# anuragranj/cc

Measured on NVIDIA H100. Metric: train-step triplets/sec at 256x832x6lvl, higher is better.
Workload: dtype f32

## Files before the change

### cc_b200/csrc/conv_tc.cu

```cuda
#include "conv.cuh"

#ifndef CCB_CPU_SIM

#include <cuda.h>
#include <cudaTypedefs.h>

namespace ccb {

constexpr int TC_M = 128;
constexpr int TC_NMAX = 128;
constexpr int TC_KC = 8;
constexpr int TC_MAX_STAGES = 4;
constexpr int TC_PRODUCERS = 128;
constexpr int TC_CONSUMER_WARPS = 8;
constexpr int TC_THREADS = TC_PRODUCERS + 32 * TC_CONSUMER_WARPS;
constexpr int TC_MAX_TAPS = 49;
constexpr int TC_PRODUCER_REGS = 72, TC_CONSUMER_REGS = 216;

struct TcArgs {
    CUtensorMap wmap;
    const float* x;
    const float* bias;
    const float* res;
    float* out;
// ... 33 lines not shown
        "}"
        : "=r"(ok)
        : "r"(smem_u32(bar)), "r"(parity)
        : "memory");
    return ok != 0;
}
__device__ __forceinline__ void mbar_wait(uint64_t* bar, uint32_t parity) {
    uint32_t spins = 0;
    while (!mbar_try(bar, parity)) {
        if (++spins > (1u << 26)) asm volatile("trap;");
    }
}
__device__ __forceinline__ void fence_proxy_async() { asm volatile("fence.proxy.async.shared::cta;" ::: "memory"); }
__device__ __forceinline__ void fence_barrier_init() { asm volatile("fence.mbarrier_init.release.cluster;" ::: "memory"); }
__device__ __forceinline__ void mbar_arrive_expect_tx(uint64_t* bar, uint32_t bytes) {
    asm volatile("mbarrier.arrive.expect_tx.shared::cta.b64 _, [%0], %1;" ::"r"(smem_u32(bar)), "r"(bytes) : "memory");
}
__device__ __forceinline__ void tma_load_3d(void* dst, const CUtensorMap* map, uint64_t* bar, int c0, int c1, int c2) {
    asm volatile(
        "cp.async.bulk.tensor.3d.shared::cluster.global.mbarrier::complete_tx::bytes [%0], [%1, {%3, %4, %5}], [%2];"
        ::"r"(smem_u32(dst)), "l"(map), "r"(smem_u32(bar)), "r"(c0), "r"(c1), "r"(c2)
        : "memory");
}
__device__ __forceinline__ void tma_prefetch_map(const CUtensorMap* map) {
    asm volatile("prefetch.tensormap [%0];" ::"l"(map) : "memory");
}
__device__ __forceinline__ void cp_async_4(uint32_t dst, const float* src, bool valid) {
    asm volatile("cp.async.ca.shared.global [%0], [%1], 4, %2;" ::"r"(dst), "l"(src), "r"(valid ? 4 : 0) : "memory");
}
__device__ __forceinline__ void cp_async_arrive(uint64_t* bar) {
    asm volatile("cp.async.mbarrier.arrive.noinc.shared::cta.b64 [%0];" ::"r"(smem_u32(bar)) : "memory");
}
__device__ __forceinline__ void cp_async_wait_all() { asm volatile("cp.async.wait_all;" ::: "memory"); }
__device__ __forceinline__ float tf32_hi(float x) {
    uint32_t r;
    asm("cvt.rna.tf32.f32 %0, %1;" : "=r"(r) : "f"(x));
    return __uint_as_float(r);
}

__device__ __forceinline__ uint64_t wg_desc(uint32_t saddr) {
    return (uint64_t)((saddr & 0x3FFFF) >> 4) | ((uint64_t)1 << 16) | ((uint64_t)(1024 >> 4) << 32) | ((uint64_t)1 << 62);
}
__device__ __forceinline__ void wg_fence() { asm volatile("wgmma.fence.sync.aligned;" ::: "memory"); }
__device__ __forceinline__ void wg_commit() { asm volatile("wgmma.commit_group.sync.aligned;" ::: "memory"); }
template <int PENDING>
__device__ __forceinline__ void wg_wait() { asm volatile("wgmma.wait_group.sync.aligned %0;" ::"n"(PENDING) : "memory"); }
template <int R>
__device__ __forceinline__ void wg_fence_regs(float (&d)[R]) {
#pragma unroll
    for (int i = 0; i < R; ++i) asm volatile("" : "+f"(d[i])::"memory");
}
template <int K, int R>
__device__ __forceinline__ void wg_fence_regs(uint32_t (&d)[K][R]) {
#pragma unroll
    for (int k = 0; k < K; ++k)
#pragma unroll
        for (int i = 0; i < R; ++i) asm volatile("" : "+r"(d[k][i])::"memory");
}

__device__ __forceinline__ void wgmma_tf32_n16(float (&d)[8], uint64_t da, uint64_t db) {
    asm volatile(
        "{\n\t.reg .pred p;\n\tsetp.ne.b32 p, 1, 0;\n\t"
        "wgmma.mma_async.sync.aligned.m64n16k8.f32.tf32.tf32 "
        "{%0, %1, %2, %3, %4, %5, %6, %7}, "
        "%8, %9, p, 1, 1;\n\t}"
        : "+f"(d[0]), "+f"(d[1]), "+f"(d[2]), "+f"(d[3]), "+f"(d[4]), "+f"(d[5]), "+f"(d[6]), "+f"(d[7])
        : "l"(da), "l"(db));
}
__device__ __forceinline__ void wgmma_tf32_n32(float (&d)[16], uint64_t da, uint64_t db) {
    asm volatile(
        "{\n\t.reg .pred p;\n\tsetp.ne.b32 p, 1, 0;\n\t"
        "wgmma.mma_async.sync.aligned.m64n32k8.f32.tf32.tf32 "
        "{%0, %1, %2, %3, %4, %5, %6, %7, %8, %9, %10, %11, %12, %13, %14, %15}, "
        "%16, %17, p, 1, 1;\n\t}"
        : "+f"(d[0]), "+f"(d[1]), "+f"(d[2]), "+f"(d[3]), "+f"(d[4]), "+f"(d[5]), "+f"(d[6]), "+f"(d[7]),
          "+f"(d[8]), "+f"(d[9]), "+f"(d[10]), "+f"(d[11]), "+f"(d[12]), "+f"(d[13]), "+f"(d[14]), "+f"(d[15])
        : "l"(da), "l"(db));
}
__device__ __forceinline__ void wgmma_tf32_n64(float (&d)[32], uint64_t da, uint64_t db) {
    asm volatile(
        "{\n\t.reg .pred p;\n\tsetp.ne.b32 p, 1, 0;\n\t"
        "wgmma.mma_async.sync.aligned.m64n64k8.f32.tf32.tf32 "
        "{%0, %1, %2, %3, %4, %5, %6, %7, %8, %9, %10, %11, %12, %13, %14, %15,"
        " %16, %17, %18, %19, %20, %21, %22, %23, %24, %25, %26, %27, %28, %29, %30, %31}, "
        "%32, %33, p, 1, 1;\n\t}"
        : "+f"(d[0]), "+f"(d[1]), "+f"(d[2]), "+f"(d[3]), "+f"(d[4]), "+f"(d[5]), "+f"(d[6]), "+f"(d[7]),
          "+f"(d[8]), "+f"(d[9]), "+f"(d[10]), "+f"(d[11]), "+f"(d[12]), "+f"(d[13]), "+f"(d[14]), "+f"(d[15]),
          "+f"(d[16]), "+f"(d[17]), "+f"(d[18]), "+f"(d[19]), "+f"(d[20]), "+f"(d[21]), "+f"(d[22]), "+f"(d[23]),
          "+f"(d[24]), "+f"(d[25]), "+f"(d[26]), "+f"(d[27]), "+f"(d[28]), "+f"(d[29]), "+f"(d[30]), "+f"(d[31])
        : "l"(da), "l"(db));
}
__device__ __forceinline__ void wgmma_tf32_n128(float (&d)[64], uint64_t da, uint64_t db) {
    asm volatile(
        "{\n\t.reg .pred p;\n\tsetp.ne.b32 p, 1, 0;\n\t"
        "wgmma.mma_async.sync.aligned.m64n128k8.f32.tf32.tf32 "
        "{%0, %1, %2, %3, %4, %5, %6, %7, %8, %9, %10, %11, %12, %13, %14, %15,"
        " %16, %17, %18, %19, %20, %21, %22, %23, %24, %25, %26, %27, %28, %29, %30, %31,"
        " %32, %33, %34, %35, %36, %37, %38, %39, %40, %41, %42, %43, %44, %45, %46, %47,"
        " %48, %49, %50, %51, %52, %53, %54, %55, %56, %57, %58, %59, %60, %61, %62, %63}, "
        "%64, %65, p, 1, 1;\n\t}"
        : "+f"(d[0]), "+f"(d[1]), "+f"(d[2]), "+f"(d[3]), "+f"(d[4]), "+f"(d[5]), "+f"(d[6]), "+f"(d[7]),
          "+f"(d[8]), "+f"(d[9]), "+f"(d[10]), "+f"(d[11]), "+f"(d[12]), "+f"(d[13]), "+f"(d[14]), "+f"(d[15]),
          "+f"(d[16]), "+f"(d[17]), "+f"(d[18]), "+f"(d[19]), "+f"(d[20]), "+f"(d[21]), "+f"(d[22]), "+f"(d[23]),
          "+f"(d[24]), "+f"(d[25]), "+f"(d[26]), "+f"(d[27]), "+f"(d[28]), "+f"(d[29]), "+f"(d[30]), "+f"(d[31]),
          "+f"(d[32]), "+f"(d[33]), "+f"(d[34]), "+f"(d[35]), "+f"(d[36]), "+f"(d[37]), "+f"(d[38]), "+f"(d[39]),
          "+f"(d[40]), "+f"(d[41]), "+f"(d[42]), "+f"(d[43]), "+f"(d[44]), "+f"(d[45]), "+f"(d[46]), "+f"(d[47]),
          "+f"(d[48]), "+f"(d[49]), "+f"(d[50]), "+f"(d[51]), "+f"(d[52]), "+f"(d[53]), "+f"(d[54]), "+f"(d[55]),
          "+f"(d[56]), "+f"(d[57]), "+f"(d[58]), "+f"(d[59]), "+f"(d[60]), "+f"(d[61]), "+f"(d[62]), "+f"(d[63])
        : "l"(da), "l"(db));
}
template <int NT>
__device__ __forceinline__ void wgmma_tf32(float (&d)[NT / 2], uint64_t da, uint64_t db) {
    if constexpr (NT == 16) wgmma_tf32_n16(d, da, db);
    else if constexpr (NT == 32) wgmma_tf32_n32(d, da, db);
    else if constexpr (NT == 64) wgmma_tf32_n64(d, da, db);
    else wgmma_tf32_n128(d, da, db);
}

__device__ __forceinline__ void wgmma_tf32_rs_n16(float (&d)[8], const uint32_t (&a)[4], uint64_t db) {
    asm volatile(
        "{\n\t.reg .pred p;\n\tsetp.ne.b32 p, 1, 0;\n\t"
        "wgmma.mma_async.sync.aligned.m64n16k8.f32.tf32.tf32 "
        "{%0, %1, %2, %3, %4, %5, %6, %7}, "
        "{%8, %9, %10, %11}, %12, p, 1, 1;\n\t}"
        : "+f"(d[0]), "+f"(d[1]), "+f"(d[2]), "+f"(d[3]), "+f"(d[4]), "+f"(d[5]), "+f"(d[6]), "+f"(d[7])
        : "r"(a[0]), "r"(a[1]), "r"(a[2]), "r"(a[3]), "l"(db));
}
__device__ __forceinline__ void wgmma_tf32_rs_n32(float (&d)[16], const uint32_t (&a)[4], uint64_t db) {
    asm volatile(
        "{\n\t.reg .pred p;\n\tsetp.ne.b32 p, 1, 0;\n\t"
        "wgmma.mma_async.sync.aligned.m64n32k8.f32.tf32.tf32 "
        "{%0, %1, %2, %3, %4, %5, %6, %7, %8, %9, %10, %11, %12, %13, %14, %15}, "
        "{%16, %17, %18, %19}, %20, p, 1, 1;\n\t}"
        : "+f"(d[0]), "+f"(d[1]), "+f"(d[2]), "+f"(d[3]), "+f"(d[4]), "+f"(d[5]), "+f"(d[6]), "+f"(d[7]),
          "+f"(d[8]), "+f"(d[9]), "+f"(d[10]), "+f"(d[11]), "+f"(d[12]), "+f"(d[13]), "+f"(d[14]), "+f"(d[15])
        : "r"(a[0]), "r"(a[1]), "r"(a[2]), "r"(a[3]), "l"(db));
}
__device__ __forceinline__ void wgmma_tf32_rs_n64(float (&d)[32], const uint32_t (&a)[4], uint64_t db) {
    asm volatile(
        "{\n\t.reg .pred p;\n\tsetp.ne.b32 p, 1, 0;\n\t"
        "wgmma.mma_async.sync.aligned.m64n64k8.f32.tf32.tf32 "
        "{%0, %1, %2, %3, %4, %5, %6, %7, %8, %9, %10, %11, %12, %13, %14, %15,"
        " %16, %17, %18, %19, %20, %21, %22, %23, %24, %25, %26, %27, %28, %29, %30, %31}, "
        "{%32, %33, %34, %35}, %36, p, 1, 1;\n\t}"
        : "+f"(d[0]), "+f"(d[1]), "+f"(d[2]), "+f"(d[3]), "+f"(d[4]), "+f"(d[5]), "+f"(d[6]), "+f"(d[7]),
          "+f"(d[8]), "+f"(d[9]), "+f"(d[10]), "+f"(d[11]), "+f"(d[12]), "+f"(d[13]), "+f"(d[14]), "+f"(d[15]),
          "+f"(d[16]), "+f"(d[17]), "+f"(d[18]), "+f"(d[19]), "+f"(d[20]), "+f"(d[21]), "+f"(d[22]), "+f"(d[23]),
          "+f"(d[24]), "+f"(d[25]), "+f"(d[26]), "+f"(d[27]), "+f"(d[28]), "+f"(d[29]), "+f"(d[30]), "+f"(d[31])
        : "r"(a[0]), "r"(a[1]), "r"(a[2]), "r"(a[3]), "l"(db));
// ... 50 lines not shown

    template <typename T>
    __device__ __forceinline__ TcTiles<T> tiles(T base, int s) const {
        const T st = base + s * stage_bytes;
        return {st, st + TC_TILE_BYTES, st + 2 * TC_TILE_BYTES, st + 2 * TC_TILE_BYTES + b_tile_bytes};
    }
    __device__ __forceinline__ TcTiles<unsigned char*> acquire(int it, int s) const {
        if (it >= depth) mbar_wait(&empty[s], ((it / depth) - 1) & 1);
        return tiles(smem, s);
    }
    __device__ __forceinline__ void publish(int s) const { fence_proxy_async(); mbar_arrive(&full[s]); }
};

__device__ __forceinline__ TcRing tc_ring(int depth, int b_tile_bytes, int full_arrivals) {
    CCB_PDL_TRIGGER();
    extern __shared__ __align__(1024) unsigned char smem_raw[];
    unsigned char* smem = smem_raw + ((1024u - (smem_u32(smem_raw) & 1023u)) & 1023u);
    const int stage_bytes = 2 * TC_TILE_BYTES + 2 * b_tile_bytes;
    uint64_t* full = (uint64_t*)(smem + depth * stage_bytes);
    const TcRing r = {smem, depth, stage_bytes, b_tile_bytes, full, full + TC_MAX_STAGES};
    if (threadIdx.x == 0) {
        for (int s = 0; s < depth; ++s) { mbar_init(&r.full[s], full_arrivals); mbar_init(&r.empty[s], TC_CONSUMER_WARPS); }
        fence_barrier_init();
    }
    __syncthreads();
    CCB_PDL_SYNC();
    return r;
}

__device__ __forceinline__ int tc_acc_row(int wg, int wq, int lane, int half) { return wg * 64 + wq * 16 + (lane >> 2) + half * 8; }
__device__ __forceinline__ int tc_acc_col(int lane, int i, int e) { return 8 * i + 2 * (lane & 3) + e; }
__device__ __forceinline__ int tc_acc_reg(int i, int half, int e) { return 4 * i + 2 * half + e; }

template <int NT>
__device__ __forceinline__ void tc_consume(const TcRing& ring, int nkt, int wg, int lane, float (&acc)[NT / 2]) {
    float part[NT / 2];
#pragma unroll
    for (int j = 0; j < NT / 2; ++j) acc[j] = 0.f;
    const uint32_t base = smem_u32(ring.smem);
    for (int it = 0; it < nkt; ++it) {
        const int s = it % ring.depth;
        mbar_wait(&ring.full[s], (it / ring.depth) & 1);
        const TcTiles<uint32_t> t = ring.tiles(base, s);
        const uint32_t a_hi = t.a_hi + wg * (TC_TILE_BYTES / 2), a_lo = t.a_lo + wg * (TC_TILE_BYTES / 2);
#pragma unroll
        for (int j = 0; j < NT / 2; ++j) part[j] = 0.f;
        wg_fence();
#pragma unroll
        for (int ks = 0; ks < TC_KC / 2; ++ks) {
            const uint32_t koff = (uint32_t)ks * 32u;
            wgmma_tf32<NT>(part, wg_desc(a_lo + koff), wg_desc(t.b_hi + koff));
            wgmma_tf32<NT>(part, wg_desc(a_hi + koff), wg_desc(t.b_lo + koff));
        }
#pragma unroll
        for (int ks = 0; ks < TC_KC / 2; ++ks) {
            const uint32_t koff = (uint32_t)ks * 32u;
            wgmma_tf32<NT>(part, wg_desc(a_hi + koff), wg_desc(t.b_hi + koff));
        }
        wg_commit();
        wg_wait<0>();
        wg_fence_regs(part);
        if (lane == 0) mbar_arrive(&ring.empty[s]);
#pragma unroll
        for (int j = 0; j < NT / 2; ++j) acc[j] += part[j];
    }
}

struct TcAFrag { uint32_t hi[TC_KC / 2][4], lo[TC_KC / 2][4]; };

__device__ __forceinline__ int tc_a_idx(int r, int k) { return k * TC_M + (r ^ (8 * (k & 3))); }
__device__ __forceinline__ int tc_a_off(int r0, int t) { return tc_a_idx(r0, t) * 4; }
__device__ __forceinline__ void tc_load_a(const unsigned char* tile, int off, float (&v)[2][8]) {
#pragma unroll
    for (int h = 0; h < 2; ++h)
#pragma unroll
        for (int j = 0; j < 8; ++j) v[h][j] = *(const float*)(tile + ((off ^ (32 * h)) + 2048 * j));
}
__device__ __forceinline__ void tc_split_a(const float (&v)[2][8], TcAFrag& f) {
#pragma unroll
    for (int ks = 0; ks < TC_KC / 2; ++ks)
#pragma unroll
        for (int i = 0; i < 4; ++i) {
            const float x = v[i & 1][2 * ks + (i >> 1)], h = tf32_hi(x);
            f.hi[ks][i] = __float_as_uint(h);
            f.lo[ks][i] = __float_as_uint(tf32_hi(x - h));
        }
}

template <int NT>
__device__ __forceinline__ void tc_consume_rs(const TcRing& ring, int g, int nkt, int wg, int wq, int lane, float (&acc)[NT / 2]) {
    constexpr bool split_ahead = NT < 128;
    float part[NT / 2];
#pragma unroll
    for (int j = 0; j < NT / 2; ++j) acc[j] = 0.f;
    const uint32_t base = smem_u32(ring.smem);
    const int a_off = tc_a_off(wg * 64 + wq * 16 + (lane >> 2), lane & 3);
    TcAFrag cur, nxt;
    float v[2][8];
    int s = g % ring.depth;
    uint32_t phase = (g / ring.depth) & 1;
    if constexpr (split_ahead) {
        if (nkt > 0) {
            mbar_wait(&ring.full[s], phase);
            tc_load_a(ring.tiles(ring.smem, s).a_hi, a_off, v);
            tc_split_a(v, cur);
        }
    }
    for (int it = 0; it < nkt; ++it) {
        if constexpr (!split_ahead) {
            mbar_wait(&ring.full[s], phase);
            tc_load_a(ring.tiles(ring.smem, s).a_hi, a_off, v);
            tc_split_a(v, cur);
        }
        const TcTiles<uint32_t> tl = ring.tiles(base, s);
#pragma unroll
        for (int j = 0; j < NT / 2; ++j) part[j] = 0.f;
        wg_fence();
#pragma unroll
        for (int ks = 0; ks < TC_KC / 2; ++ks) {
            const uint32_t koff = (uint32_t)ks * 32u;
            wgmma_tf32_rs<NT>(part, cur.lo[ks], wg_desc(tl.b_hi + koff));
            wgmma_tf32_rs<NT>(part, cur.hi[ks], wg_desc(tl.b_lo + koff));
        }
#pragma unroll
        for (int ks = 0; ks < TC_KC / 2; ++ks)
            wgmma_tf32_rs<NT>(part, cur.hi[ks], wg_desc(tl.b_hi + (uint32_t)ks * 32u));
        wg_commit();
        const int s1 = s + 1 == ring.depth ? 0 : s + 1;
        const uint32_t phase1 = phase ^ (s1 == 0);
        if constexpr (split_ahead) {
            if (it + 1 < nkt) {
                mbar_wait(&ring.full[s1], phase1);
                tc_load_a(ring.tiles(ring.smem, s1).a_hi, a_off, v);
                tc_split_a(v, nxt);
            }
        }
        wg_wait<0>();
        wg_fence_regs(part);
        wg_fence_regs(cur.hi);
        wg_fence_regs(cur.lo);
        if (lane == 0) mbar_arrive(&ring.empty[s]);
#pragma unroll
        for (int j = 0; j < NT / 2; ++j) acc[j] += part[j];
        if constexpr (split_ahead) cur = nxt;
        s = s1;
        phase = phase1;
    }
}

struct TcUnit { int m0, n0, z, kt_beg, nkt; };
__device__ __forceinline__ TcUnit tc_unit(const TcArgs& a, int u) {
    TcUnit w;
    w.m0 = (u % a.tiles_m) * TC_M;
    u /= a.tiles_m;
    w.n0 = (u % a.tiles_n) * TC_NMAX;
    w.z = u / a.tiles_n;
    w.kt_beg = w.z * a.kt_per_split;
    w.nkt = max(0, min(a.ktiles, w.kt_beg + a.kt_per_split) - w.kt_beg);
    return w;
}

template <int NT>
__global__ void __launch_bounds__(TC_THREADS, 1) conv_tc_kernel(const __grid_constant__ TcArgs a) {
    const TcRing ring = tc_ring(a.depth, a.b_tile_bytes, TC_PRODUCERS + 1);
    const int tid = threadIdx.x, warp = tid >> 5, lane = tid & 31;
    const long long HWin = (long long)a.Hin * a.Win;

    if (warp < TC_PRODUCERS / 32) {
        wg_regs_dec<TC_PRODUCER_REGS>();
        const int r = tid;
        const int cpt = a.cpad >> 2;
        const int nchunks = a.ntaps * cpt;
        if (r == 0) tma_prefetch_map(&a.wmap);
        int g = 0;
        for (int u = blockIdx.x; u < a.units; u += gridDim.x) {
            const TcUnit w = tc_unit(a, u);
            const int m = w.m0 + r;
            const bool mvalid = m < a.M;
            int b = 0, oy = 0, ox = 0;
            if (mvalid) {
                int hw = a.Hc * a.Wc;
                b = m / hw;
                int rem = m - b * hw;
                oy = rem / a.Wc;
// ... 35 lines not shown
#pragma unroll
                    for (int c = 0; c < TC_KC; ++c) {
                        const float* p = a.x;
                        int nv = 0;
                        if (mvalid && q < nchunks) {
                            const int iy = iy0 + a.off_y[tap], ix = ix0 + a.off_x[tap];
                            if (iy >= 0 && iy < a.Hin && ix >= 0 && ix < a.Win) {
                                p = xb + (long long)(c4 * 4) * HWin + (iy * a.Win + ix);
                                nv = a.Cin - c4 * 4;
                            }
                        }
#pragma unroll
                        for (int j = 0; j < 4; ++j) {
                            const bool v = j < nv;
                            cp_async_4(at + 4 * tc_a_idx(r, 4 * c + j), v ? p + j * HWin : a.x, v);
                        }
                        ++q;
                        if (++c4 == cpt) { c4 = 0; ++tap; }
                    }
                }
                cp_async_arrive(&ring.full[s]);
            }
        }
        cp_async_wait_all();
    } else {
        wg_regs_inc<TC_CONSUMER_REGS>();
        const int wg = (warp - TC_PRODUCERS / 32) >> 2, wq = warp & 3;
        const long long HWout = (long long)a.Hout * a.Wout;
        int g = 0;
        for (int u = blockIdx.x; u < a.units; u += gridDim.x) {
            const TcUnit w = tc_unit(a, u);
            const int ntile = min(TC_NMAX, a.Ntot - w.n0);
            float acc[NT / 2];
            tc_consume_rs<NT>(ring, g, w.nkt, wg, wq, lane, acc);
            g += w.nkt;
#pragma unroll
            for (int half = 0; half < 2; ++half) {
                const int em = w.m0 + tc_acc_row(wg, wq, lane, half);
                if (em >= a.M) continue;
                int hw = a.Hc * a.Wc;
                int eb = em / hw;
                int rem = em - eb * hw;
                int eoy = rem / a.Wc, eox = rem - eoy * a.Wc;
                const long long obase = (long long)eb * a.Ntot * HWout + (long long)(eoy * a.out_stride + a.out_oy) * a.Wout +
                                        (eox * a.out_stride + a.out_ox);
#pragma unroll
                for (int i = 0; i < NT / 8; ++i)
#pragma unroll
                    for (int e = 0; e < 2; ++e) {
                        const int nl = tc_acc_col(lane, i, e);
                        if (nl < ntile) {
                            float o = acc[tc_acc_reg(i, half, e)];
                            const int n = w.n0 + nl;
                            const long long off = obase + (long long)n * HWout;
                            if (a.splits > 1) {
                                a.partial[(long long)w.z * a.out_numel + off] = o;
                            } else {
                                if (a.bias) o += __ldg(a.bias + n);
                                if (a.res) o += __ldg(a.res + off);
                                a.out[off] = apply_act(o, a.act, a.slope);
                            }
                        }
                    }
            }
        }
    }
}
// ... 13 lines not shown
}

template <typename Args>
static int tc_launch_kernel(void (*const (&kfns)[4])(const Args), const Args& a, int nt, dim3 grid, int smem, cudaStream_t st,
                            const char* what) {
    auto kfn = kfns[nt == 16 ? 0 : nt == 32 ? 1 : nt == 64 ? 2 : 3];
    cudaFuncSetAttribute(kfn, cudaFuncAttributeMaxDynamicSharedMemorySize, TC_SMEM_MAX);
    CCB_LAUNCH(kfn, grid, dim3(TC_THREADS), smem, st, a);
    return check_launch(what);
}

static void (*const TC_FPROP_KERNELS[4])(const TcArgs) = {conv_tc_kernel<16>, conv_tc_kernel<32>, conv_tc_kernel<64>,
                                                          conv_tc_kernel<128>};

static int tc_weight_map(CUtensorMap* map, const float* wp, int N, int Kp, int nt) {
    static PFN_cuTensorMapEncodeTiled_v12000 encode = [] {
        void* fn = nullptr;
        cudaDriverEntryPointQueryResult q;
        if (cudaGetDriverEntryPointByVersion("cuTensorMapEncodeTiled", &fn, 12000, cudaEnableDefault, &q) != cudaSuccess ||
            q != cudaDriverEntryPointSuccess)
            fn = nullptr;
        return (PFN_cuTensorMapEncodeTiled_v12000)fn;
    }();
    CCB_REQUIRE(encode, CCB_ERR_LAUNCH, "conv_tc: the driver has no cuTensorMapEncodeTiled");
    const cuuint64_t dims[3] = {(cuuint64_t)Kp, (cuuint64_t)N, 2};
    const cuuint64_t strides[2] = {(cuuint64_t)Kp * sizeof(float), (cuuint64_t)N * Kp * sizeof(float)};
    const cuuint32_t box[3] = {TC_KC * 4, (cuuint32_t)nt, 1};
    const cuuint32_t estrides[3] = {1, 1, 1};
    const CUresult rc = encode(map, CU_TENSOR_MAP_DATA_TYPE_FLOAT32, 3, (void*)wp, dims, strides, box, estrides,
                               CU_TENSOR_MAP_INTERLEAVE_NONE, CU_TENSOR_MAP_SWIZZLE_128B, CU_TENSOR_MAP_L2_PROMOTION_L2_256B,
                               CU_TENSOR_MAP_FLOAT_OOB_FILL_NONE);
    CCB_REQUIRE(rc == CUDA_SUCCESS, CCB_ERR_LAUNCH, "conv_tc: cuTensorMapEncodeTiled failed (%d) for N %d Kp %d", (int)rc, N, Kp);
    return CCB_OK;
}

static int launch_tc(TcArgs& a, const float* w, int mode, int N, int Cc, int KK, int Ci, const signed char* tap_index,
                     float* wp, float* partial, int splits, cudaStream_t st) {
    a.cpad = roundup(Cc, 4);
    a.Kp = tc_kp(a.ntaps, Cc);
    WPrepDesc p;
    memset(&p, 0, sizeof(p));
    p.w = w; p.wp = wp; p.N = N; p.Cc = Cc; p.KK = KK; p.ntaps = a.ntaps; p.Kp = a.Kp; p.mode = mode; p.Ci = Ci;
    p.layout = WPREP_TC; p.p0 = a.cpad;
    for (int t = 0; t < a.ntaps; ++t) p.tap_index[t] = tap_index[t];
    const float* wpp = nullptr;
    int rc = wprep_get(p, st, &wpp);
    if (rc) return rc;
    a.Ntot = N;
    a.splits = splits;
    a.ktiles = a.Kp / (TC_KC * 4);
    a.kt_per_split = cdiv(a.ktiles, splits);
    a.partial = partial;
    int nt, smem;
    tc_geometry(N, nt, a.b_tile_bytes, a.depth, smem);
    rc = tc_weight_map(&a.wmap, wpp, N, a.Kp, nt);
    if (rc) return rc;
    a.tiles_m = cdiv(a.M, TC_M);
    a.tiles_n = cdiv(N, TC_NMAX);
    a.units = a.tiles_m * a.tiles_n * splits;
    static int sms = [] {
        int dev = 0, n = 0;
        cudaGetDevice(&dev);
        cudaDeviceGetAttribute(&n, cudaDevAttrMultiProcessorCount, dev);
        return n > 0 ? n : NUM_SMS;
    }();
    return tc_launch_kernel(TC_FPROP_KERNELS, a, nt, dim3(a.units < sms ? a.units : sms), smem, st, "conv_tc");
}

struct TcWgradArgs {
    const float* x;
    const float* dy;
    float* out;
    int B, Ci, Hi, Wi, Co, Ho, Wo, kh, kw, stride, pad;
    int cpad, Mtot;
    int P;
    int ktiles, kt_per_split, splits;
    int depth, b_tile_bytes;
};

template <int NT>
__global__ void __launch_bounds__(TC_THREADS, 1) conv_tc_wgrad_kernel(const TcWgradArgs a) {
    const TcRing ring = tc_ring(a.depth, a.b_tile_bytes, TC_PRODUCERS);
    const int tid = threadIdx.x, warp = tid >> 5, lane = tid & 31;
    const int m0 = blockIdx.x * TC_M, n0 = blockIdx.y * TC_NMAX;
    const int ntile = min(TC_NMAX, a.Co - n0);
    const int kt_beg = blockIdx.z * a.kt_per_split;
    const int nkt = min(a.ktiles, kt_beg + a.kt_per_split) - kt_beg;
    const int KK = a.kh * a.kw;
    const int HWo = a.Ho * a.Wo, HWi = a.Hi * a.Wi;

    if (warp < TC_PRODUCERS / 32) {
        const int c = tid & 7, rbase = tid >> 3;
        int rowoff[8], dky[8], dkx[8];
        unsigned rvalid = 0;
#pragma unroll
        for (int j = 0; j < 8; ++j) {
            int m = m0 + rbase + 16 * j;
            rowoff[j] = 0; dky[j] = dkx[j] = 0;
            if (m < a.Mtot) {
                int tap = m / a.cpad, ci = m - tap * a.cpad;
                if (ci < a.Ci) {
                    int ky = tap / a.kw, kx = tap - ky * a.kw;
                    dky[j] = ky - a.pad; dkx[j] = kx - a.pad;
                    rowoff[j] = ci * HWi + dky[j] * a.Wi + dkx[j];
                    rvalid |= 1u << j;
                }
            }
        }
        for (int it = 0; it < nkt; ++it) {
            const int s = it % ring.depth;
            const int p0 = ((kt_beg + it) * TC_KC + c) * 4;
            const bool pvalid = p0 < a.P;
            int b = 0, oy = 0, ox0 = 0;
            if (pvalid) {
                b = p0 / HWo;
                int rem = p0 - b * HWo;
                oy = rem / a.Wo;
                ox0 = rem - oy * a.Wo;
            }
            const float* xpix = a.x + (long long)b * a.Ci * HWi + (oy * a.stride) * a.Wi + ox0 * a.stride;
            const int iyb = oy * a.stride, ixb = ox0 * a.stride;
            float av[8][4];
            float4 bv[8];
#pragma unroll
            for (int j = 0; j < 8; ++j) {
                av[j][0] = av[j][1] = av[j][2] = av[j][3] = 0.f;
                const int iy = iyb + dky[j], ix0 = ixb + dkx[j];
                if (pvalid && ((rvalid >> j) & 1u) && iy >= 0 && iy < a.Hi) {
                    const float* px = xpix + rowoff[j];
                    if (ix0 >= 0 && ix0 + 3 * a.stride < a.Wi) {
#pragma unroll
                        for (int e = 0; e < 4; ++e) av[j][e] = __ldg(px + e * a.stride);
                    } else {
#pragma unroll
                        for (int e = 0; e < 4; ++e) {
                            const int ix = ix0 + e * a.stride;
                            if (ix >= 0 && ix < a.Wi) av[j][e] = __ldg(px + e * a.stride);
                        }
                    }
                }
                bv[j] = make_float4(0.f, 0.f, 0.f, 0.f);
                const int n = rbase + 16 * j;
                if (pvalid && n < ntile)
                    bv[j] = __ldg((const float4*)(a.dy + ((long long)b * a.Co + n0 + n) * HWo + oy * a.Wo + ox0));
            }
            const TcTiles<unsigned char*> t = ring.acquire(it, s);
#pragma unroll
            for (int j = 0; j < 8; ++j) {
                const int r = rbase + 16 * j, idx = tile_idx(r, c);
                tc_split_store(t.a_hi, t.a_lo, idx, make_float4(av[j][0], av[j][1], av[j][2], av[j][3]));
                if (r < NT) tc_split_store(t.b_hi, t.b_lo, idx, bv[j]);
            }
            ring.publish(s);
        }
    } else {
        const int wg = (warp - TC_PRODUCERS / 32) >> 2, wq = warp & 3;
        float acc[NT / 2];
        tc_consume<NT>(ring, nkt, wg, lane, acc);
        float* outp = a.out + (long long)blockIdx.z * a.Co * a.Ci * KK;
#pragma unroll
        for (int half = 0; half < 2; ++half) {
            const int em = m0 + tc_acc_row(wg, wq, lane, half);
            if (em >= a.Mtot) continue;
            const int etap = em / a.cpad;
            const int eci = em - etap * a.cpad;
            if (eci >= a.Ci) continue;
#pragma unroll
            for (int i = 0; i < NT / 8; ++i)
#pragma unroll
                for (int e = 0; e < 2; ++e) {
                    const int nl = tc_acc_col(lane, i, e);
                    if (nl < ntile) outp[((long long)(n0 + nl) * a.Ci + eci) * KK + etap] = acc[tc_acc_reg(i, half, e)];
                }
        }
    }
}

static void (*const TC_WGRAD_KERNELS[4])(const TcWgradArgs) = {conv_tc_wgrad_kernel<16>, conv_tc_wgrad_kernel<32>,
                                                                conv_tc_wgrad_kernel<64>, conv_tc_wgrad_kernel<128>};

bool tc_supported(const ccb_conv_desc* d, int op) {
    if (d->kh != d->kw || d->kh * d->kw > TC_MAX_TAPS) return false;
    if (op == CCB_CONV_WGRAD) return (d->Wo % 4 == 0);
    return true;
}
bool tc_profitable(const ccb_conv_desc* d, int op) {
    if (!tc_supported(d, op)) return false;
    const long long M = (op == CCB_CONV_FPROP) ? (long long)d->B * d->Ho * d->Wo : (long long)d->B * d->Hi * d->Wi;
    const long long wsize = (long long)d->Ci * d->Co * d->kh * d->kw;
    return (M >= 128 && wsize >= 64) || (M >= 8 && wsize >= 65536);
}

int tc_plan(const ccb_conv_desc* d, int op, long long& panel_floats) {
    panel_floats = 0;
    if (op == CCB_CONV_WGRAD) {
        const int ktiles = cdiv(d->B * d->Ho * d->Wo, 32);
        const int tiles = cdiv(d->kh * d->kw * roundup(d->Ci, 4), TC_M) * cdiv(d->Co, TC_NMAX);
        int splits = cdiv(2 * NUM_SMS, tiles);
        if (splits > ktiles / 4) splits = ktiles / 4;
        if (splits > 2 * NUM_SMS) splits = 2 * NUM_SMS;
        if (splits < 1) splits = 1;
        return cdiv(ktiles, cdiv(ktiles, splits));
    }
    const bool fp = op == CCB_CONV_FPROP;
    const int s = fp ? 1 : d->stride, N = fp ? d->Co : d->Ci;
    const int Kp = tc_kp(cdiv(d->kh, s) * cdiv(d->kw, s), fp ? d->Ci : d->Co);
// ... 56 lines not shown
            for (int ty = 0; ty < k.nky; ++ty)
                for (int tx = 0; tx < k.nkx; ++tx) {
                    const int ky = k.ky0 + ty * s, kx = k.kx0 + tx * s, t = ty * k.nkx + tx;
                    a.off_y[t] = (signed char)((py + d->pad - ky) / s);
                    a.off_x[t] = (signed char)((px + d->pad - kx) / s);
                    tix[t] = (signed char)(ky * d->kw + kx);
                }
            int rc = launch_tc(a, w, 1, d->Ci, d->Co, d->kh * d->kw, d->Ci, tix, wp, partial, splits, st);
            if (rc) return rc;
        }
    if (splits > 1) {
        launch_splitk_reduce(partial, dx, bias, res, out_numel, splits, d->Hi * d->Wi, d->Ci, d->act, d->slope, st);
        return check_launch("conv_tc dgrad splitk reduce");
    }
    return CCB_OK;
}

int tc_wgrad(const ccb_conv_desc* d, const float* x, const float* dy, float* dw, float* partial, int splits, cudaStream_t st) {
    TcWgradArgs a;
    memset(&a, 0, sizeof(a));
    a.x = x; a.dy = dy;
    a.B = d->B; a.Ci = d->Ci; a.Hi = d->Hi; a.Wi = d->Wi; a.Co = d->Co; a.Ho = d->Ho; a.Wo = d->Wo;
    a.kh = d->kh; a.kw = d->kw; a.stride = d->stride; a.pad = d->pad;
    a.cpad = roundup(d->Ci, 4);
    a.Mtot = d->kh * d->kw * a.cpad;
    a.P = d->B * d->Ho * d->Wo;
    a.ktiles = cdiv(a.P, 32);
    a.kt_per_split = cdiv(a.ktiles, splits);
    a.splits = splits;
    a.out = splits > 1 ? partial : dw;
    const long long numel = (long long)d->Co * d->Ci * d->kh * d->kw;
    int nt, wsmem;
    tc_geometry(d->Co, nt, a.b_tile_bytes, a.depth, wsmem);
    dim3 grid(cdiv(a.Mtot, TC_M), cdiv(d->Co, TC_NMAX), a.splits);
    int rc = tc_launch_kernel(TC_WGRAD_KERNELS, a, nt, grid, wsmem, st, "conv_tc_wgrad");
    if (rc || a.splits == 1) return rc;
    launch_splitk_reduce(partial, dw, nullptr, nullptr, numel, splits, 1, 1, CCB_ACT_NONE, 0.f, st);
    return check_launch("conv_tc_wgrad_reduce");
}

}

extern "C" int ccb_debug_tc_plan(int N, int* out4) {
    if (N < 1 || !out4) return CCB_ERR_ARG;
    ccb::tc_geometry(N, out4[0], out4[1], out4[2], out4[3]);
    return CCB_OK;
}

#else

namespace ccb {
bool tc_supported(const ccb_conv_desc*, int) { return false; }
bool tc_profitable(const ccb_conv_desc*, int) { return false; }
int tc_plan(const ccb_conv_desc*, int, long long& panel_floats) { panel_floats = 0; return 1; }
int tc_fprop(const ccb_conv_desc*, const float*, const float*, const float*, const float*, float*, float*, float*, int,
             cudaStream_t) { return CCB_ERR_UNSUPPORTED; }
int tc_dgrad(const ccb_conv_desc*, const float*, const float*, const float*, const float*, float*, float*, float*, int,
             cudaStream_t) { return CCB_ERR_UNSUPPORTED; }
int tc_wgrad(const ccb_conv_desc*, const float*, const float*, float*, float*, int, cudaStream_t) { return CCB_ERR_UNSUPPORTED; }
}

extern "C" int ccb_debug_tc_plan(int, int*) { return CCB_ERR_UNSUPPORTED; }

#endif
```

Measured before the change: 57.89.

## Make wgrad TC kernel persistent with cp.async producers and register-sourced A splitting

```diff
diff --git a/cc_b200/csrc/conv_tc.cu b/cc_b200/csrc/conv_tc.cu
--- a/cc_b200/csrc/conv_tc.cu
+++ b/cc_b200/csrc/conv_tc.cu
@@ -89,6 +89,9 @@
     asm volatile("cp.async.mbarrier.arrive.noinc.shared::cta.b64 [%0];" ::"r"(smem_u32(bar)) : "memory");
 }
 __device__ __forceinline__ void cp_async_wait_all() { asm volatile("cp.async.wait_all;" ::: "memory"); }
+__device__ __forceinline__ void cp_async_16(uint32_t dst, const void* src, bool valid) {
+    asm volatile("cp.async.cg.shared.global [%0], [%1], 16, %2;" ::"r"(dst), "l"(src), "r"(valid ? 16 : 0) : "memory");
+}
 __device__ __forceinline__ float tf32_hi(float x) {
     uint32_t r;
     asm("cvt.rna.tf32.f32 %0, %1;" : "=r"(r) : "f"(x));
@@ -113,65 +116,6 @@
     for (int k = 0; k < K; ++k)
 #pragma unroll
         for (int i = 0; i < R; ++i) asm volatile("" : "+r"(d[k][i])::"memory");
-}
-
-__device__ __forceinline__ void wgmma_tf32_n16(float (&d)[8], uint64_t da, uint64_t db) {
-    asm volatile(
-        "{\n\t.reg .pred p;\n\tsetp.ne.b32 p, 1, 0;\n\t"
-        "wgmma.mma_async.sync.aligned.m64n16k8.f32.tf32.tf32 "
-        "{%0, %1, %2, %3, %4, %5, %6, %7}, "
-        "%8, %9, p, 1, 1;\n\t}"
-        : "+f"(d[0]), "+f"(d[1]), "+f"(d[2]), "+f"(d[3]), "+f"(d[4]), "+f"(d[5]), "+f"(d[6]), "+f"(d[7])
-        : "l"(da), "l"(db));
-}
-__device__ __forceinline__ void wgmma_tf32_n32(float (&d)[16], uint64_t da, uint64_t db) {
-    asm volatile(
-        "{\n\t.reg .pred p;\n\tsetp.ne.b32 p, 1, 0;\n\t"
-        "wgmma.mma_async.sync.aligned.m64n32k8.f32.tf32.tf32 "
-        "{%0, %1, %2, %3, %4, %5, %6, %7, %8, %9, %10, %11, %12, %13, %14, %15}, "
-        "%16, %17, p, 1, 1;\n\t}"
-        : "+f"(d[0]), "+f"(d[1]), "+f"(d[2]), "+f"(d[3]), "+f"(d[4]), "+f"(d[5]), "+f"(d[6]), "+f"(d[7]),
-          "+f"(d[8]), "+f"(d[9]), "+f"(d[10]), "+f"(d[11]), "+f"(d[12]), "+f"(d[13]), "+f"(d[14]), "+f"(d[15])
-        : "l"(da), "l"(db));
-}
-__device__ __forceinline__ void wgmma_tf32_n64(float (&d)[32], uint64_t da, uint64_t db) {
-    asm volatile(
-        "{\n\t.reg .pred p;\n\tsetp.ne.b32 p, 1, 0;\n\t"
-        "wgmma.mma_async.sync.aligned.m64n64k8.f32.tf32.tf32 "
-        "{%0, %1, %2, %3, %4, %5, %6, %7, %8, %9, %10, %11, %12, %13, %14, %15,"
-        " %16, %17, %18, %19, %20, %21, %22, %23, %24, %25, %26, %27, %28, %29, %30, %31}, "
-        "%32, %33, p, 1, 1;\n\t}"
-        : "+f"(d[0]), "+f"(d[1]), "+f"(d[2]), "+f"(d[3]), "+f"(d[4]), "+f"(d[5]), "+f"(d[6]), "+f"(d[7]),
-          "+f"(d[8]), "+f"(d[9]), "+f"(d[10]), "+f"(d[11]), "+f"(d[12]), "+f"(d[13]), "+f"(d[14]), "+f"(d[15]),
-          "+f"(d[16]), "+f"(d[17]), "+f"(d[18]), "+f"(d[19]), "+f"(d[20]), "+f"(d[21]), "+f"(d[22]), "+f"(d[23]),
-          "+f"(d[24]), "+f"(d[25]), "+f"(d[26]), "+f"(d[27]), "+f"(d[28]), "+f"(d[29]), "+f"(d[30]), "+f"(d[31])
-        : "l"(da), "l"(db));
-}
-__device__ __forceinline__ void wgmma_tf32_n128(float (&d)[64], uint64_t da, uint64_t db) {
-    asm volatile(
-        "{\n\t.reg .pred p;\n\tsetp.ne.b32 p, 1, 0;\n\t"
-        "wgmma.mma_async.sync.aligned.m64n128k8.f32.tf32.tf32 "
-        "{%0, %1, %2, %3, %4, %5, %6, %7, %8, %9, %10, %11, %12, %13, %14, %15,"
-        " %16, %17, %18, %19, %20, %21, %22, %23, %24, %25, %26, %27, %28, %29, %30, %31,"
-        " %32, %33, %34, %35, %36, %37, %38, %39, %40, %41, %42, %43, %44, %45, %46, %47,"
-        " %48, %49, %50, %51, %52, %53, %54, %55, %56, %57, %58, %59, %60, %61, %62, %63}, "
-        "%64, %65, p, 1, 1;\n\t}"
-        : "+f"(d[0]), "+f"(d[1]), "+f"(d[2]), "+f"(d[3]), "+f"(d[4]), "+f"(d[5]), "+f"(d[6]), "+f"(d[7]),
-          "+f"(d[8]), "+f"(d[9]), "+f"(d[10]), "+f"(d[11]), "+f"(d[12]), "+f"(d[13]), "+f"(d[14]), "+f"(d[15]),
-          "+f"(d[16]), "+f"(d[17]), "+f"(d[18]), "+f"(d[19]), "+f"(d[20]), "+f"(d[21]), "+f"(d[22]), "+f"(d[23]),
-          "+f"(d[24]), "+f"(d[25]), "+f"(d[26]), "+f"(d[27]), "+f"(d[28]), "+f"(d[29]), "+f"(d[30]), "+f"(d[31]),
-          "+f"(d[32]), "+f"(d[33]), "+f"(d[34]), "+f"(d[35]), "+f"(d[36]), "+f"(d[37]), "+f"(d[38]), "+f"(d[39]),
-          "+f"(d[40]), "+f"(d[41]), "+f"(d[42]), "+f"(d[43]), "+f"(d[44]), "+f"(d[45]), "+f"(d[46]), "+f"(d[47]),
-          "+f"(d[48]), "+f"(d[49]), "+f"(d[50]), "+f"(d[51]), "+f"(d[52]), "+f"(d[53]), "+f"(d[54]), "+f"(d[55]),
-          "+f"(d[56]), "+f"(d[57]), "+f"(d[58]), "+f"(d[59]), "+f"(d[60]), "+f"(d[61]), "+f"(d[62]), "+f"(d[63])
-        : "l"(da), "l"(db));
-}
-template <int NT>
-__device__ __forceinline__ void wgmma_tf32(float (&d)[NT / 2], uint64_t da, uint64_t db) {
-    if constexpr (NT == 16) wgmma_tf32_n16(d, da, db);
-    else if constexpr (NT == 32) wgmma_tf32_n32(d, da, db);
-    else if constexpr (NT == 64) wgmma_tf32_n64(d, da, db);
-    else wgmma_tf32_n128(d, da, db);
 }
 
 __device__ __forceinline__ void wgmma_tf32_rs_n16(float (&d)[8], const uint32_t (&a)[4], uint64_t db) {
@@ -288,49 +232,24 @@
 __device__ __forceinline__ int tc_acc_col(int lane, int i, int e) { return 8 * i + 2 * (lane & 3) + e; }
 __device__ __forceinline__ int tc_acc_reg(int i, int half, int e) { return 4 * i + 2 * half + e; }
 
-template <int NT>
-__device__ __forceinline__ void tc_consume(const TcRing& ring, int nkt, int wg, int lane, float (&acc)[NT / 2]) {
-    float part[NT / 2];
-#pragma unroll
-    for (int j = 0; j < NT / 2; ++j) acc[j] = 0.f;
-    const uint32_t base = smem_u32(ring.smem);
-    for (int it = 0; it < nkt; ++it) {
-        const int s = it % ring.depth;
-        mbar_wait(&ring.full[s], (it / ring.depth) & 1);
-        const TcTiles<uint32_t> t = ring.tiles(base, s);
-        const uint32_t a_hi = t.a_hi + wg * (TC_TILE_BYTES / 2), a_lo = t.a_lo + wg * (TC_TILE_BYTES / 2);
-#pragma unroll
-        for (int j = 0; j < NT / 2; ++j) part[j] = 0.f;
-        wg_fence();
-#pragma unroll
-        for (int ks = 0; ks < TC_KC / 2; ++ks) {
-            const uint32_t koff = (uint32_t)ks * 32u;
-            wgmma_tf32<NT>(part, wg_desc(a_lo + koff), wg_desc(t.b_hi + koff));
-            wgmma_tf32<NT>(part, wg_desc(a_hi + koff), wg_desc(t.b_lo + koff));
-        }
-#pragma unroll
-        for (int ks = 0; ks < TC_KC / 2; ++ks) {
-            const uint32_t koff = (uint32_t)ks * 32u;
-            wgmma_tf32<NT>(part, wg_desc(a_hi + koff), wg_desc(t.b_hi + koff));
-        }
-        wg_commit();
-        wg_wait<0>();
-        wg_fence_regs(part);
-        if (lane == 0) mbar_arrive(&ring.empty[s]);
-#pragma unroll
-        for (int j = 0; j < NT / 2; ++j) acc[j] += part[j];
-    }
-}
-
 struct TcAFrag { uint32_t hi[TC_KC / 2][4], lo[TC_KC / 2][4]; };
 
 __device__ __forceinline__ int tc_a_idx(int r, int k) { return k * TC_M + (r ^ (8 * (k & 3))); }
-__device__ __forceinline__ int tc_a_off(int r0, int t) { return tc_a_idx(r0, t) * 4; }
+struct TcAFprop {
+    __device__ __forceinline__ static int off(int r0, int t) { return tc_a_idx(r0, t) * 4; }
+    __device__ __forceinline__ static int at(int off, int h, int j) { return (off ^ (32 * h)) + 2048 * j; }
+};
+struct TcAWgrad {
+    __device__ __forceinline__ static int idx(int r, int k) { return 32 * r + (k ^ (4 * (r & 7))); }
+    __device__ __forceinline__ static int off(int r0, int t) { return idx(r0, t) * 4; }
+    __device__ __forceinline__ static int at(int off, int h, int j) { return (off + 1024 * h) ^ (16 * j); }
+};
+template <typename L>
 __device__ __forceinline__ void tc_load_a(const unsigned char* tile, int off, float (&v)[2][8]) {
 #pragma unroll
     for (int h = 0; h < 2; ++h)
 #pragma unroll
-        for (int j = 0; j < 8; ++j) v[h][j] = *(const float*)(tile + ((off ^ (32 * h)) + 2048 * j));
+        for (int j = 0; j < 8; ++j) v[h][j] = *(const float*)(tile + L::at(off, h, j));
 }
 __device__ __forceinline__ void tc_split_a(const float (&v)[2][8], TcAFrag& f) {
 #pragma unroll
@@ -343,31 +262,42 @@
         }
 }
 
-template <int NT>
-__device__ __forceinline__ void tc_consume_rs(const TcRing& ring, int g, int nkt, int wg, int wq, int lane, float (&acc)[NT / 2]) {
+__device__ __forceinline__ void tc_consumer_sync() { asm volatile("bar.sync 1, %0;" ::"n"(32 * TC_CONSUMER_WARPS) : "memory"); }
+
+struct TcFpropFeed {
+    static constexpr bool split_b = false;
+    __device__ __forceinline__ void prep_b(const TcTiles<unsigned char*>&) const {}
+};
+
+template <int NT, typename L, typename Feed>
+__device__ __forceinline__ void tc_consume_rs(const TcRing& ring, int g, int nkt, int wg, int wq, int lane, const Feed& feed,
+                                              float (&acc)[NT / 2]) {
     constexpr bool split_ahead = NT < 128;
-    float part[NT / 2];
 #pragma unroll
     for (int j = 0; j < NT / 2; ++j) acc[j] = 0.f;
     const uint32_t base = smem_u32(ring.smem);
-    const int a_off = tc_a_off(wg * 64 + wq * 16 + (lane >> 2), lane & 3);
+    const int a_off = L::off(wg * 64 + wq * 16 + (lane >> 2), lane & 3);
     TcAFrag cur, nxt;
-    float v[2][8];
+    auto take = [&](int st, uint32_t ph, TcAFrag& f) {
+        mbar_wait(&ring.full[st], ph);
+        const TcTiles<unsigned char*> t = ring.tiles(ring.smem, st);
+        float v[2][8];
+        tc_load_a<L>(t.a_hi, a_off, v);
+        tc_split_a(v, f);
+        if constexpr (Feed::split_b) {
+            feed.prep_b(t);
+            fence_proxy_async();
+            tc_consumer_sync();
+        }
+    };
+    float part[NT / 2];
     int s = g % ring.depth;
     uint32_t phase = (g / ring.depth) & 1;
     if constexpr (split_ahead) {
-        if (nkt > 0) {
-            mbar_wait(&ring.full[s], phase);
-            tc_load_a(ring.tiles(ring.smem, s).a_hi, a_off, v);
-            tc_split_a(v, cur);
-        }
+        if (nkt > 0) take(s, phase, cur);
     }
     for (int it = 0; it < nkt; ++it) {
-        if constexpr (!split_ahead) {
-            mbar_wait(&ring.full[s], phase);
-            tc_load_a(ring.tiles(ring.smem, s).a_hi, a_off, v);
-            tc_split_a(v, cur);
-        }
+        if constexpr (!split_ahead) take(s, phase, cur);
         const TcTiles<uint32_t> tl = ring.tiles(base, s);
 #pragma unroll
         for (int j = 0; j < NT / 2; ++j) part[j] = 0.f;
@@ -385,11 +315,7 @@
         const int s1 = s + 1 == ring.depth ? 0 : s + 1;
         const uint32_t phase1 = phase ^ (s1 == 0);
         if constexpr (split_ahead) {
-            if (it + 1 < nkt) {
-                mbar_wait(&ring.full[s1], phase1);
-                tc_load_a(ring.tiles(ring.smem, s1).a_hi, a_off, v);
-                tc_split_a(v, nxt);
-            }
+            if (it + 1 < nkt) take(s1, phase1, nxt);
         }
         wg_wait<0>();
         wg_fence_regs(part);
@@ -405,7 +331,8 @@
 }
 
 struct TcUnit { int m0, n0, z, kt_beg, nkt; };
-__device__ __forceinline__ TcUnit tc_unit(const TcArgs& a, int u) {
+template <typename Args>
+__device__ __forceinline__ TcUnit tc_unit(const Args& a, int u) {
     TcUnit w;
     w.m0 = (u % a.tiles_m) * TC_M;
     u /= a.tiles_m;
@@ -507,7 +434,7 @@
             const TcUnit w = tc_unit(a, u);
             const int ntile = min(TC_NMAX, a.Ntot - w.n0);
             float acc[NT / 2];
-            tc_consume_rs<NT>(ring, g, w.nkt, wg, wq, lane, acc);
+            tc_consume_rs<NT, TcAFprop>(ring, g, w.nkt, wg, wq, lane, TcFpropFeed(), acc);
             g += w.nkt;
 #pragma unroll
             for (int half = 0; half < 2; ++half) {
@@ -587,6 +514,16 @@
                                CU_TENSOR_MAP_FLOAT_OOB_FILL_NONE);
     CCB_REQUIRE(rc == CUDA_SUCCESS, CCB_ERR_LAUNCH, "conv_tc: cuTensorMapEncodeTiled failed (%d) for N %d Kp %d", (int)rc, N, Kp);
     return CCB_OK;
+}
+
+static dim3 tc_persistent_grid(int units) {
+    static int sms = [] {
+        int dev = 0, n = 0;
+        cudaGetDevice(&dev);
+        cudaDeviceGetAttribute(&n, cudaDevAttrMultiProcessorCount, dev);
+        return n > 0 ? n : NUM_SMS;
+    }();
+    return dim3(units < sms ? units : sms);
 }
 
 static int launch_tc(TcArgs& a, const float* w, int mode, int N, int Cc, int KK, int Ci, const signed char* tap_index,
@@ -613,13 +550,7 @@
     a.tiles_m = cdiv(a.M, TC_M);
     a.tiles_n = cdiv(N, TC_NMAX);
     a.units = a.tiles_m * a.tiles_n * splits;
-    static int sms = [] {
-        int dev = 0, n = 0;
-        cudaGetDevice(&dev);
-        cudaDeviceGetAttribute(&n, cudaDevAttrMultiProcessorCount, dev);
-        return n > 0 ? n : NUM_SMS;
-    }();
-    return tc_launch_kernel(TC_FPROP_KERNELS, a, nt, dim3(a.units < sms ? a.units : sms), smem, st, "conv_tc");
+    return tc_launch_kernel(TC_FPROP_KERNELS, a, nt, tc_persistent_grid(a.units), smem, st, "conv_tc");
 }
 
 struct TcWgradArgs {
@@ -630,103 +561,131 @@
     int cpad, Mtot;
     int P;
     int ktiles, kt_per_split, splits;
+    int tiles_m, tiles_n, units;
     int depth, b_tile_bytes;
+};
+
+template <int NT>
+struct TcWgradFeed {
+    static constexpr bool split_b = true;
+    int ct;
+    __device__ __forceinline__ void prep_b(const TcTiles<unsigned char*>& t) const {
+        constexpr int n4 = NT * TC_KC, nthr = 32 * TC_CONSUMER_WARPS;
+#pragma unroll
+        for (int i = 0; i < (n4 + nthr - 1) / nthr; ++i) {
+            const int q = ct + nthr * i;
+            if (n4 % nthr == 0 || q < n4) tc_split_store(t.b_hi, t.b_lo, q, ((const float4*)t.a_lo)[q]);
+        }
+    }
 };
 
 template <int NT>
 __global__ void __launch_bounds__(TC_THREADS, 1) conv_tc_wgrad_kernel(const TcWgradArgs a) {
     const TcRing ring = tc_ring(a.depth, a.b_tile_bytes, TC_PRODUCERS);
     const int tid = threadIdx.x, warp = tid >> 5, lane = tid & 31;
-    const int m0 = blockIdx.x * TC_M, n0 = blockIdx.y * TC_NMAX;
-    const int ntile = min(TC_NMAX, a.Co - n0);
-    const int kt_beg = blockIdx.z * a.kt_per_split;
-    const int nkt = min(a.ktiles, kt_beg + a.kt_per_split) - kt_beg;
-    const int KK = a.kh * a.kw;
     const int HWo = a.Ho * a.Wo, HWi = a.Hi * a.Wi;
 
     if (warp < TC_PRODUCERS / 32) {
-        const int c = tid & 7, rbase = tid >> 3;
-        int rowoff[8], dky[8], dkx[8];
-        unsigned rvalid = 0;
-#pragma unroll
-        for (int j = 0; j < 8; ++j) {
-            int m = m0 + rbase + 16 * j;
-            rowoff[j] = 0; dky[j] = dkx[j] = 0;
-            if (m < a.Mtot) {
-                int tap = m / a.cpad, ci = m - tap * a.cpad;
-                if (ci < a.Ci) {
-                    int ky = tap / a.kw, kx = tap - ky * a.kw;
-                    dky[j] = ky - a.pad; dkx[j] = kx - a.pad;
-                    rowoff[j] = ci * HWi + dky[j] * a.Wi + dkx[j];
-                    rvalid |= 1u << j;
-                }
+        wg_regs_dec<TC_PRODUCER_REGS>();
+        const int c = tid & 7, n_lo = tid >> 3, dy_idx = tile_idx(n_lo, c);
+        static_assert(1023 + 2 * TC_MAX_STAGES * 8 + TC_PRODUCERS / 32 * 8 * 8 <= 2048, "row-group table past the ring");
+        int2* const gtab = (int2*)(ring.empty + TC_MAX_STAGES) + 8 * warp;
+        int g = 0;
+        for (int u = blockIdx.x; u < a.units; u += gridDim.x) {
+            const TcUnit w = tc_unit(a, u);
+            const int ntile = min(TC_NMAX, a.Co - w.n0);
+            __syncwarp();
+            if (lane < 8) {
+                const int m = w.m0 + 32 * warp + 4 * lane;
+                const int tap = m / a.cpad, ci = m - tap * a.cpad, ky = tap / a.kw, kx = tap - ky * a.kw;
+                const int nv = m < a.Mtot ? max(0, min(4, a.Ci - ci)) : 0;
+                gtab[lane] = make_int2(ci * HWi + ky * a.Wi + kx, ky | kx << 8 | nv << 16);
             }
-        }
-        for (int it = 0; it < nkt; ++it) {
-            const int s = it % ring.depth;
-            const int p0 = ((kt_beg + it) * TC_KC + c) * 4;
-            const bool pvalid = p0 < a.P;
-            int b = 0, oy = 0, ox0 = 0;
-            if (pvalid) {
-                b = p0 / HWo;
-                int rem = p0 - b * HWo;
-                oy = rem / a.Wo;
-                ox0 = rem - oy * a.Wo;
-            }
-            const float* xpix = a.x + (long long)b * a.Ci * HWi + (oy * a.stride) * a.Wi + ox0 * a.stride;
-            const int iyb = oy * a.stride, ixb = ox0 * a.stride;
-            float av[8][4];
-            float4 bv[8];
-#pragma unroll
-            for (int j = 0; j < 8; ++j) {
-                av[j][0] = av[j][1] = av[j][2] = av[j][3] = 0.f;
-                const int iy = iyb + dky[j], ix0 = ixb + dkx[j];
-                if (pvalid && ((rvalid >> j) & 1u) && iy >= 0 && iy < a.Hi) {
-                    const float* px = xpix + rowoff[j];
-                    if (ix0 >= 0 && ix0 + 3 * a.stride < a.Wi) {
-#pragma unroll
-                        for (int e = 0; e < 4; ++e) av[j][e] = __ldg(px + e * a.stride);
+            __syncwarp();
+            int p = w.kt_beg * (TC_KC * 4) + lane;
+            int b = p / HWo, oy = (p - b * HWo) / a.Wo, ox = p - b * HWo - oy * a.Wo;
+            const float* dyn = a.dy + (long long)(w.n0 + n_lo) * HWo;
+            for (int it = 0; it < w.nkt; ++it, ++g) {
+                const int s = g % ring.depth;
+                const TcTiles<unsigned char*> t = ring.acquire(g, s);
+                const bool pvalid = p < a.P;
+                const int iy0 = oy * a.stride - a.pad, ix0 = ox * a.stride - a.pad, pix = iy0 * a.Wi + ix0;
+                const float* xb = a.x + (pvalid ? (long long)b * a.Ci * HWi : 0ll);
+                asm("" : "+l"(xb));
+                uint32_t ab[8];
+#pragma unroll
+                for (int k = 0; k < 8; ++k) ab[k] = (smem_u32(t.a_hi) + 4096 * warp + 4 * lane) ^ (16 * k);
+                int2 gh[4];
+#pragma unroll
+                for (int q = 0; q < 8; ++q) {
+                    if (q % 4 == 0) {
+#pragma unroll
+                        for (int i = 0; i < 4; ++i) gh[i] = gtab[q + i];
+                    }
+                    const int2 gq = gh[q % 4];
+                    const int ky = gq.y & 0xff, kx = (gq.y >> 8) & 0xff, nv = gq.y >> 16;
+                    const bool ok = pvalid && (unsigned)(iy0 + ky) < (unsigned)a.Hi && (unsigned)(ix0 + kx) < (unsigned)a.Wi;
+                    const int o = pix + gq.x;
+                    if (nv == 4) {
+                        const float* src = xb + (ok ? o : 0);
+                        const int step = ok ? HWi : 0;
+#pragma unroll
+                        for (int e = 0; e < 4; ++e)
+                            cp_async_4(ab[(4 * q + e) % 8] + 128 * (4 * q + e), src + e * step, ok);
                     } else {
+                        const int n = ok ? nv : 0;
 #pragma unroll
                         for (int e = 0; e < 4; ++e) {
-                            const int ix = ix0 + e * a.stride;
-                            if (ix >= 0 && ix < a.Wi) av[j][e] = __ldg(px + e * a.stride);
+                            const bool v = e < n;
+                            cp_async_4(ab[(4 * q + e) % 8] + 128 * (4 * q + e), xb + (v ? o + e * HWi : 0), v);
                         }
                     }
                 }
-                bv[j] = make_float4(0.f, 0.f, 0.f, 0.f);
-                const int n = rbase + 16 * j;
-                if (pvalid && n < ntile)
-                    bv[j] = __ldg((const float4*)(a.dy + ((long long)b * a.Co + n0 + n) * HWo + oy * a.Wo + ox0));
+                const int p0 = p - lane;
+                const int bc = __shfl_sync(0xffffffffu, b, 4 * c), remc = __shfl_sync(0xffffffffu, oy * a.Wo + ox, 4 * c);
+                const bool cvalid = p0 + 4 * c < a.P;
+                const float* dyc = dyn + (long long)bc * a.Co * HWo + remc;
+                const uint32_t bt = smem_u32(t.a_lo) + 16 * dy_idx;
+#pragma unroll
+                for (int j = 0; j < NT / 16; ++j) {
+                    const bool v = cvalid && n_lo + 16 * j < ntile;
+                    cp_async_16(bt + 2048 * j, v ? dyc + (long long)(16 * j) * HWo : a.dy, v);
+                }
+                p += TC_KC * 4;
+                for (ox += TC_KC * 4; ox >= a.Wo; ox -= a.Wo)
+                    if (++oy == a.Ho) { oy = 0; ++b; }
+                cp_async_arrive(&ring.full[s]);
             }
-            const TcTiles<unsigned char*> t = ring.acquire(it, s);
-#pragma unroll
-            for (int j = 0; j < 8; ++j) {
-                const int r = rbase + 16 * j, idx = tile_idx(r, c);
-                tc_split_store(t.a_hi, t.a_lo, idx, make_float4(av[j][0], av[j][1], av[j][2], av[j][3]));
-                if (r < NT) tc_split_store(t.b_hi, t.b_lo, idx, bv[j]);
+        }
+        cp_async_wait_all();
+    } else {
+        wg_regs_inc<TC_CONSUMER_REGS>();
+        const int wg = (warp - TC_PRODUCERS / 32) >> 2, wq = warp & 3;
+        const int KK = a.kh * a.kw;
+        const TcWgradFeed<NT> feed = {tid - TC_PRODUCERS};
+        int g = 0;
+        for (int u = blockIdx.x; u < a.units; u += gridDim.x) {
+            const TcUnit w = tc_unit(a, u);
+            const int ntile = min(TC_NMAX, a.Co - w.n0);
+            float acc[NT / 2];
+            tc_consume_rs<NT, TcAWgrad>(ring, g, w.nkt, wg, wq, lane, feed, acc);
+            g += w.nkt;
+            float* outp = a.out + (long long)w.z * a.Co * a.Ci * KK;
+#pragma unroll
+            for (int half = 0; half < 2; ++half) {
+                const int em = w.m0 + tc_acc_row(wg, wq, lane, half);
+                if (em >= a.Mtot) continue;
+                const int etap = em / a.cpad;
+                const int eci = em - etap * a.cpad;
+                if (eci >= a.Ci) continue;
+#pragma unroll
+                for (int i = 0; i < NT / 8; ++i)
+#pragma unroll
+                    for (int e = 0; e < 2; ++e) {
+                        const int nl = tc_acc_col(lane, i, e);
+                        if (nl < ntile) outp[((long long)(w.n0 + nl) * a.Ci + eci) * KK + etap] = acc[tc_acc_reg(i, half, e)];
+                    }
             }
-            ring.publish(s);
-        }
-    } else {
-        const int wg = (warp - TC_PRODUCERS / 32) >> 2, wq = warp & 3;
-        float acc[NT / 2];
-        tc_consume<NT>(ring, nkt, wg, lane, acc);
-        float* outp = a.out + (long long)blockIdx.z * a.Co * a.Ci * KK;
-#pragma unroll
-        for (int half = 0; half < 2; ++half) {
-            const int em = m0 + tc_acc_row(wg, wq, lane, half);
-            if (em >= a.Mtot) continue;
-            const int etap = em / a.cpad;
-            const int eci = em - etap * a.cpad;
-            if (eci >= a.Ci) continue;
-#pragma unroll
-            for (int i = 0; i < NT / 8; ++i)
-#pragma unroll
-                for (int e = 0; e < 2; ++e) {
-                    const int nl = tc_acc_col(lane, i, e);
-                    if (nl < ntile) outp[((long long)(n0 + nl) * a.Ci + eci) * KK + etap] = acc[tc_acc_reg(i, half, e)];
-                }
         }
     }
 }
@@ -849,8 +808,10 @@
     const long long numel = (long long)d->Co * d->Ci * d->kh * d->kw;
     int nt, wsmem;
     tc_geometry(d->Co, nt, a.b_tile_bytes, a.depth, wsmem);
-    dim3 grid(cdiv(a.Mtot, TC_M), cdiv(d->Co, TC_NMAX), a.splits);
-    int rc = tc_launch_kernel(TC_WGRAD_KERNELS, a, nt, grid, wsmem, st, "conv_tc_wgrad");
+    a.tiles_m = cdiv(a.Mtot, TC_M);
+    a.tiles_n = cdiv(d->Co, TC_NMAX);
+    a.units = a.tiles_m * a.tiles_n * splits;
+    int rc = tc_launch_kernel(TC_WGRAD_KERNELS, a, nt, tc_persistent_grid(a.units), wsmem, st, "conv_tc_wgrad");
     if (rc || a.splits == 1) return rc;
     launch_splitk_reduce(partial, dw, nullptr, nullptr, numel, splits, 1, 1, CCB_ACT_NONE, 0.f, st);
     return check_launch("conv_tc_wgrad_reduce");
```

Measured after the change: 64.64 (median of 6 runs). 1.12x the previous value.
